# ankitkumar93/compute-war

Measured on AMD Instinct MI355X. Metric: GB/s ingested (Skein-512 + LZ4, 64 KiB blocks), higher is better.
Workload: dtype u64; 1 GPU; skein512+lz4, 1048576 x 65536 B uniform-random blocks/GPU in HBM; blocks_per_gpu=1048576, block_bytes=65536, parallelism=block-sharded x1, gather-only RCCL

## Files before the change

compute_war_amd/csrc/lz4_kernel.hip:

```cpp

#include <hip/hip_runtime.h>
#include <stdint.h>
#include <stdio.h>
#include <stdlib.h>
#include <string.h>

#include <mutex>
#include <type_traits>
#include <unordered_map>

#include "cw_device.h"
#include "lz_device.h"

#ifndef HEADW_GLOBAL
#define HEADW_GLOBAL 16
#endif
#ifndef HEADW_STAGED
#define HEADW_STAGED 64
#endif

namespace cw {

using lz::Around;
using lz::around;
// ... 188 lines not shown
struct Chunk { uint4 p[kPieces]; };

__device__ __forceinline__ void chunk_load(Chunk &r, const uint8_t *g, uint32_t c, uint32_t nchunks, uint32_t n, uint32_t lane)
{
#pragma unroll
    for (uint32_t j = 0; j < kPieces; j++) {
        const uint32_t off = c * kChunk + j * 1024 + lane * 16;
        if (c < nchunks && off < n) r.p[j] = *reinterpret_cast<const uint4 *>(g + off);
    }
}
__device__ __forceinline__ void chunk_stage(const Chunk &r, uint32_t *ring32, uint32_t c, uint32_t n, uint32_t lane)
{
#pragma unroll
    for (uint32_t j = 0; j < kPieces; j++) {
        const uint32_t off = c * kChunk + j * 1024 + lane * 16;
        if (off < n) *reinterpret_cast<uint4 *>(reinterpret_cast<uint8_t *>(ring32) + (off & (kRing - 1))) = r.p[j];
    }
}
__device__ __forceinline__ void chunk_store(const Chunk &r, uint8_t *lit, uint32_t c, uint32_t n, uint32_t lane)
{
#pragma unroll
    for (uint32_t j = 0; j < kPieces; j++) {
        const uint32_t off = c * kChunk + j * 1024 + lane * 16;
        if (off < n) {
            uint32_t *q = reinterpret_cast<uint32_t *>(lit + off);
            __builtin_nontemporal_store(r.p[j].x, q);
            __builtin_nontemporal_store(r.p[j].y, q + 1);
            __builtin_nontemporal_store(r.p[j].z, q + 2);
            __builtin_nontemporal_store(r.p[j].w, q + 3);
        }
    }
}

struct Walk {
    ScanState st;
    uint32_t knext = 0, v0 = 0;
    bool marked = false;
};

template <int NG>
__device__ __forceinline__ void probe_groups(Walk &w, const uint32_t (&pos)[kStreamGroup], const bool (&act)[kStreamGroup], uint32_t *tab,
                                             const uint32_t *ring32, uint32_t tag, uint32_t epoch)
{
    uint32_t v[NG], old[NG];
#pragma unroll
    for (int j = 0; j < NG; j++) {
        const uint32_t a0 = (pos[j] & (kRing - 1)) >> 2, a1 = (a0 + 1) & (kRing / 4 - 1);
        v[j] = __builtin_amdgcn_alignbyte(ring32[a1], ring32[a0], pos[j] & 3u);
    }
#pragma unroll
    for (int j = 0; j < NG; j++) old[j] = scan_issue(tab, tag, pos[j], v[j], act[j]);
#pragma unroll
    for (int j = 0; j < NG; j++) scan_judge(old[j], epoch, w.v0, pos[j], v[j], act[j], w.st);
}

__device__ __forceinline__ void probe_upto(Walk &w, uint32_t end, uint32_t *tab, const uint32_t *ring32, uint32_t tag, uint32_t epoch,
                                           uint32_t nprobes, const uint8_t *g, uint32_t lane)
{
    for (;;) {
        uint32_t pos[kStreamGroup], nact = 0, ngroups = 0;
        bool act[kStreamGroup];
#pragma unroll
        for (uint32_t j = 0; j < kStreamGroup; j++) {
            const uint32_t k = w.knext + 64 * j + lane;
            pos[j] = 1 + probe_delta(k);
            act[j] = k < nprobes && pos[j] < end;
            const unsigned long long m = __ballot(act[j]);
            nact += (uint32_t)__builtin_popcountll(m);
            ngroups += m != 0;
        }
        if (nact == 0) return;
        if (ngroups == 1) probe_groups<1>(w, pos, act, tab, ring32, tag, epoch);
        else if (ngroups == 2) probe_groups<2>(w, pos, act, tab, ring32, tag, epoch);
        else probe_groups<kStreamGroup>(w, pos, act, tab, ring32, tag, epoch);
        w.marked = scan_settle(g, w.st);
        w.knext += nact;
        if (w.marked || nact < 64 * kStreamGroup) return;
    }
}

__global__ void __launch_bounds__(64)
lz4_scan_stream_kernel(const uint8_t *__restrict__ src, uint32_t n, size_t src_stride, size_t nblocks,
                       uint8_t *__restrict__ dst, size_t dst_stride, uint32_t *__restrict__ sizes, uint32_t nprobes,
                       uint32_t *__restrict__ queue, uint32_t *__restrict__ counters, size_t first_block, uint32_t feed_word)
{
    __shared__ __attribute__((aligned(16))) uint32_t tab[1u << 13];
    __shared__ __attribute__((aligned(16))) uint32_t ring32[kRing / 4];
    volatile uint32_t *mailbox = ring32;
    const uint32_t lane = threadIdx.x;
    __builtin_amdgcn_s_setprio(3);
    uint32_t epoch = 15;
    const uint32_t nchunks = (n + kChunk - 1) / kChunk;
    const uint32_t hdr = 1 + (n >= 15 ? (n - 15) / 255 + 1 : 0);

    BlockFeed feed;
    const uint32_t run = n >= 65536 ? 1u : 65536u / n;
    for (size_t rel; scan_next_block(feed, rel, counters + feed_word - 2, mailbox, run, nblocks - first_block, lane);) {
        const size_t blk = first_block + rel;
        scan_begin_block(tab, epoch, lane);
        const uint8_t *g = src + blk * src_stride;
        uint8_t *out = dst + blk * dst_stride, *lit = out + hdr;
        const uint32_t tag = epoch << 28;
        Walk w;
        Chunk r0, r1, r2;

#define CW_STAGE(PREV, CUR, C)                                                                         \
        do {                                                                                           \
            const uint32_t c_ = (C);                                                                   \
            if (c_) chunk_store(PREV, lit, c_ - 1, n, lane);                                           \
            chunk_load(PREV, g, c_ + 2, nchunks, n, lane);                                             \
            chunk_stage(CUR, ring32, c_, n, lane);                                                     \
            if (c_ == 0) {                                                                             \
                w.v0 = ring32[0];                                                                      \
                if (nprobes && lane == 0) {                                                            \
                    const uint32_t h0 = w.v0 * 2654435761u;                                            \
                    atomicMax(&tab[h0 >> 19], tag | ((h0 >> 7) & 0xFFFu));             \
                }                                                                                      \
            } else {                                                                                   \
                probe_upto(w, c_ * kChunk, tab, ring32, tag, epoch, nprobes, g, lane);                 \
            }                                                                                          \
        } while (0)

        chunk_load(r0, g, 0, nchunks, n, lane);
        chunk_load(r1, g, 1, nchunks, n, lane);
        for (uint32_t c = 0; c < nchunks && !w.marked; c += 3) {
            CW_STAGE(r2, r0, c);
            if (c + 1 < nchunks && !w.marked) CW_STAGE(r0, r1, c + 1);
            if (c + 2 < nchunks && !w.marked) CW_STAGE(r1, r2, c + 2);
        }
#undef CW_STAGE
        if (!w.marked) {
            probe_upto(w, n, tab, ring32, tag, epoch, nprobes, g, lane);
            if (!w.marked) {
                const uint32_t last = (nchunks - 1) % 3;
                if (last == 0) chunk_store(r0, lit, nchunks - 1, n, lane);
                else if (last == 1) chunk_store(r1, lit, nchunks - 1, n, lane);
                else chunk_store(r2, lit, nchunks - 1, n, lane);
            }
        }
        if (w.marked) {
            scan_mark(sizes, blk, queue, counters, lane);
            continue;
        }
        if (n >= 15) {
            if (lane == 0) out[0] = 15u << 4;
            put_len(out + 1, n - 15, lane);
        } else if (lane == 0) {
            out[0] = (uint8_t)(n << 4);
        }
        if (lane == 0) sizes[blk] = hdr + n;
    }
}

#ifdef CW_CLOCK_STAMP
__device__ unsigned long long g_clock_scan[4 * kClockSlots];
hipError_t lz4_clock_read(unsigned long long *out) { return hipMemcpyFromSymbol(out, HIP_SYMBOL(g_clock_scan), sizeof g_clock_scan); }
#endif

__global__ void __launch_bounds__(64)
lz4_scan_span_kernel(const uint8_t *__restrict__ src, uint32_t n, size_t src_stride, uint32_t nspans, uint8_t *__restrict__ dst,
                     size_t dst_stride, uint32_t *__restrict__ sizes, uint32_t nprobes, uint32_t *__restrict__ queue,
                     uint32_t *__restrict__ counters, uint32_t lg)
{
    CW_CLOCK_SCOPE(g_clock_scan);
    __shared__ __attribute__((aligned(16))) uint32_t tab[1u << 13];
    __shared__ __attribute__((aligned(16))) uint32_t ring32[kRing / 4];
    volatile uint32_t *mailbox = ring32;
    const uint32_t lane = threadIdx.x;
    __builtin_amdgcn_s_setprio(3);
    uint32_t epoch = 15;
    const uint32_t cmask = (1u << lg) - 1, run = 16u >> lg;
    const uint32_t hdr = 1 + (n - 15) / 255 + 1;
    const uint32_t lane16 = lane * 16;

    for (;;) {
        __syncthreads();
        if (lane == 0) *mailbox = atomicAdd(&counters[2], 1u);
        __syncthreads();
        const uint32_t span = __builtin_amdgcn_readfirstlane(*mailbox);
        if (span >= nspans) break;
        __syncthreads();
        const size_t first = (size_t)span * run;
        const uint8_t *gs = src + first * src_stride;
        uint8_t *os = dst + first * dst_stride + hdr;

        Walk w;
        size_t blk = first;
        uint32_t tag = 0, marks = 0;
        Chunk r0, r1, r2;
#define CW_LD(R, I)                                                                                          \
        do {                                                                                                 \
            const uint32_t i_ = (I) < 15u ? (I) : 15u;                                                       \
            const uint8_t *p_ = gs + (size_t)(i_ >> lg) * src_stride + ((i_ & cmask) << 12) + lane16;        \
            _Pragma("unroll") for (uint32_t j = 0; j < kPieces; j++) R.p[j] = *reinterpret_cast<const uint4 *>(p_ + j * 1024); \
        } while (0)
#define CW_ST(R, I)                                                                                          \
        do {                                                                                                 \
            const uint32_t i_ = (I);                                                                         \
            uint8_t *p_ = os + (size_t)(i_ >> lg) * dst_stride + ((i_ & cmask) << 12) + lane16;              \
            _Pragma("unroll") for (uint32_t j = 0; j < kPieces; j++) {                                       \
                uint32_t *q = reinterpret_cast<uint32_t *>(p_ + j * 1024);  \
                __builtin_nontemporal_store(R.p[j].x, q);     __builtin_nontemporal_store(R.p[j].y, q + 1);  \
                __builtin_nontemporal_store(R.p[j].z, q + 2); __builtin_nontemporal_store(R.p[j].w, q + 3);  \
            }                                                                                                \
        } while (0)
#define CW_FINISH()                                                                                          \
        do {                      \
            if (!w.marked) probe_upto(w, n, tab, ring32, tag, epoch, nprobes, src + blk * src_stride, lane); \
            if (w.marked) marks |= 1u << (uint32_t)(blk - first);         \
            else {                                                                                           \
                uint8_t *out = dst + blk * dst_stride;                                                       \
                if (lane == 0) out[0] = 15u << 4;                                                            \
                put_len(out + 1, n - 15, lane);                                                              \
                if (lane == 0) sizes[blk] = hdr + n;                                                         \
            }                                                                                                \
        } while (0)
#define CW_BEGIN(I)                                                                                          \
        do {                                                                                                 \
            blk = first + ((I) >> lg);                                                                       \
            scan_begin_block(tab, epoch, lane);                                                              \
            tag = epoch << 28;                                                                               \
            w = Walk();                                                                                      \
        } while (0)
#define CW_STAGE_IN(R, C)                                                                                    \
        do {                                                                                                 \
            uint8_t *p_ = reinterpret_cast<uint8_t *>(ring32) + (((C) & 1u) << 12) + lane16;                 \
            _Pragma("unroll") for (uint32_t j = 0; j < kPieces; j++) *reinterpret_cast<uint4 *>(p_ + j * 1024) = R.p[j]; \
        } while (0)
#define CW_AFTER_STAGE(C)                                                                                    \
        do {                                                                                                 \
            if ((C) == 0) {                                                                                  \
                w.v0 = ring32[0];                                                                            \
                if (nprobes && lane == 0) {                                                                  \
                    const uint32_t h0 = w.v0 * 2654435761u;                                                  \
                    atomicMax(&tab[h0 >> 19], tag | ((h0 >> 7) & 0xFFFu));                   \
                }                                                                                            \
            } else if (!w.marked) {                                                                          \
                probe_upto(w, (C) * kChunk, tab, ring32, tag, epoch, nprobes, src + blk * src_stride, lane); \
            }                                                                                                \
        } while (0)
#define CW_STEP(PREV, CUR, I)                                                                                \
        do {                                                                                                 \
            const uint32_t s_ = (I), c_ = s_ & cmask;                                                        \
            CW_ST(PREV, s_ - 1);                                                                             \
            CW_LD(PREV, s_ + 2);                                                                             \
            if (c_ == 0) { CW_FINISH(); CW_BEGIN(s_); }                                                      \
            CW_STAGE_IN(CUR, c_);                                                                            \
            CW_AFTER_STAGE(c_);                                                                              \
        } while (0)

        CW_LD(r0, 0u);
        CW_LD(r1, 1u);
        CW_LD(r2, 2u);
        CW_BEGIN(0u);
        CW_STAGE_IN(r0, 0u);
        CW_AFTER_STAGE(0u);
        for (uint32_t i = 1; i < 16; i += 3) {
            CW_STEP(r0, r1, i);
            CW_STEP(r1, r2, i + 1);
            CW_STEP(r2, r0, i + 2);
        }
        CW_ST(r0, 15u);
        CW_FINISH();
        if (marks) {
            uint32_t base = 0;
            if (lane == 0) base = atomicAdd(&counters[1], (uint32_t)__builtin_popcount(marks));
            base = __builtin_amdgcn_readfirstlane(base);
            if (lane < 16 && ((marks >> lane) & 1u)) {
                sizes[first + lane] = kNeedsParse;
                queue[base + (uint32_t)__builtin_popcount(marks & ((1u << lane) - 1u))] = (uint32_t)(first + lane);
            }
        }
#undef CW_LD
#undef CW_ST
#undef CW_FINISH
#undef CW_BEGIN
#undef CW_STAGE_IN
#undef CW_AFTER_STAGE
#undef CW_STEP
    }
}

static uint32_t scan_probes(uint32_t n)
{
    if (n < kMFLimit + 1) return 0;
    const uint32_t limit = n - 11;
    uint32_t k = 0, p = 1, step = 1, nb = 64;
    while (p + step <= limit) { p += step; step = nb++ >> 6; k++; }
    return k;
}

template <bool STAGED>
__global__ void __launch_bounds__(64)
lz4_blocks_kernel(const uint8_t *__restrict__ src, uint32_t n, size_t src_stride, size_t nblocks,
                  uint8_t *__restrict__ dst, size_t dst_stride, uint32_t *__restrict__ sizes,
                  const uint32_t *__restrict__ queue, uint32_t *__restrict__ counters)
{
    extern __shared__ __attribute__((aligned(16))) uint8_t smem[];
    uint16_t *tab = reinterpret_cast<uint16_t *>(smem);
    uint8_t *lds_in = smem + kTabBytes;
    const uint32_t lane = threadIdx.x;

    const uint32_t qcount = counters[1];
    volatile uint32_t *mailbox = reinterpret_cast<volatile uint32_t *>(tab);
    for (uint32_t guard = 0; guard <= qcount; guard++) {
        __syncthreads();
        if (lane == 0) *mailbox = atomicAdd(&counters[0], 1u);
        __syncthreads();
        const uint32_t qi = __builtin_amdgcn_readfirstlane(*mailbox);
        if (qi >= qcount) break;
        const size_t blk = queue[qi];
        const uint8_t *g = src + blk * src_stride;
        uint8_t *out = dst + blk * dst_stride;

        __syncthreads();
        const uint8_t *in = STAGED ? lds_in : g;
        if (STAGED) {
            if ((reinterpret_cast<uintptr_t>(g) & 15) == 0) {
                const uint4 *g4 = reinterpret_cast<const uint4 *>(g);
                const uint32_t nvec = n >> 4;
                for (uint32_t i = lane; i < nvec; i += 64) reinterpret_cast<uint4 *>(lds_in)[i] = g4[i];
                for (uint32_t i = (nvec << 4) + lane; i < n; i += 64) lds_in[i] = g[i];
            } else {
                for (uint32_t i = lane; i < n; i += 64) lds_in[i] = g[i];
            }
        }
        for (uint32_t i = lane; i < kTabBytes / 16; i += 64) reinterpret_cast<uint4 *>(tab)[i] = make_uint4(0, 0, 0, 0);
        __syncthreads();

        uint32_t ip = 0, anchor = 0, op = 0;

        if (n >= kMFLimit + 1) {
            const uint32_t mflimit = n - kMFLimit, matchlimit = n - kLastLiterals;
            uint32_t ins = 0, s0 = 1;
            bool has_retest = false;

            for (uint32_t seq = 0; seq < n; seq++) {
                uint32_t match = 0, mpos = 0;
                bool found = false, exhausted = false;
                for (uint32_t t0 = 0;;) {
                    const uint32_t t = t0 + lane, k = t - 2;
                    const bool is_probe = t >= 2;
                    const uint32_t dk = t0 == 0 ? k : probe_delta(k), stepk = k == 0 ? 1u : (63u + k) >> 6;
                    const uint32_t pos = t == 0 ? ins : t == 1 ? ip : s0 + dk;
                    const bool dead = is_probe && s0 + dk + stepk > mflimit + 1;
                    const bool active = !dead && (is_probe || t == 0 || has_retest);
                    const uint32_t ndead = ctz64(__ballot(dead));
                    const unsigned long long amask = __ballot(active);
                    if (!amask) { exhausted = true; break; }

                    uint32_t v = 0, h = 0, old = 0;
                    if (active) {
                        v = rd32x<STAGED>(in, pos);
                        h = hash13(v);
                        old = tab[h];
                        tab[h] = (uint16_t)pos;
                    }
                    __syncthreads();
                    const bool lost = active && (tab[h] != (uint16_t)pos);
                    const uint32_t fa = ctz64(amask);
                    uint32_t m = ctz64(__ballot(lost));
                    if (m == fa) m = fa + 1;
                    const uint32_t L = m < ndead ? m : ndead;

                    const bool eq = active && t != 0 && lane < L && rd32x<STAGED>(in, old) == v;
                    const unsigned long long eqmask = __ballot(eq);
                    const uint32_t ncommit = eqmask ? ctz64(eqmask) + 1 : L;
                    if (__ballot(active && lane >= ncommit)) {
                        if (active && lane >= ncommit) tab[h] = (uint16_t)old;
                        if (active && lane < ncommit) tab[h] = (uint16_t)pos;
                    }
                    if (eqmask) {
                        const uint32_t w = ctz64(eqmask);
                        mpos = __builtin_amdgcn_readlane(pos, w);
                        match = __builtin_amdgcn_readlane(old, w);
                        found = true;
                        break;
                    }
                    if (ndead < 64 && L == ndead) { exhausted = true; break; }
                    t0 += L;
                }
                (void)exhausted;
                if (!found) break;
                ip = mpos;

                uint32_t mc, back;
                {
                    bool ok;
                    if (lane < 48) {
                        const uint32_t i = ip + kMinMatch + lane;
                        ok = i < matchlimit && in[i] == in[match + kMinMatch + lane];
// ... 1083 lines not shown
            state = LB_NEXT;
        }
    }
}

template <int K>
__global__ void __launch_bounds__(64)
lz4_lanes_ring_kernel(const uint8_t *__restrict__ src, uint32_t n, size_t src_stride, uint8_t *__restrict__ dst, size_t dst_stride,
                      uint32_t *__restrict__ sizes, const uint32_t *__restrict__ queue, uint32_t *__restrict__ counters,
                      uint16_t *__restrict__ tables, uint32_t min_blocks, uint32_t reserve, uint32_t max_blocks)
{
    __shared__ uint32_t ring[(kRingBytes / 4) * 64];
    const uint32_t qcount = counters[1];
    if (qcount < min_blocks || qcount >= max_blocks) return;
    if ((size_t)blockIdx.x * 64 >= qcount) return;
    lz4_lanes_ring_body<K>(ring, qcount, src, n, src_stride, dst, dst_stride, sizes, queue, counters, tables, reserve);
}

__global__ void __launch_bounds__(64)
lz4_lanes_ring_auto_kernel(const uint8_t *__restrict__ src, uint32_t n, size_t src_stride, uint8_t *__restrict__ dst, size_t dst_stride,
                           uint32_t *__restrict__ sizes, const uint32_t *__restrict__ queue, uint32_t *__restrict__ counters,
                           uint16_t *__restrict__ tables, uint32_t min_blocks, uint32_t reserve_mid, uint32_t wide_from, uint32_t reserve_wide,
                           uint32_t leave_mid)
{
    __shared__ uint32_t ring[(kRingBytes / 4) * 64];
    const uint32_t qcount = counters[1];
    if (qcount < min_blocks) return;
    if ((size_t)blockIdx.x * 64 >= qcount) return;
    if (qcount >= wide_from) {
        lz4_lanes_ring_body<1>(ring, qcount, src, n, src_stride, dst, dst_stride, sizes, queue, counters, tables, reserve_wide);
    } else {
        if ((size_t)blockIdx.x * 64 + leave_mid >= qcount && blockIdx.x > 0) return;
        lz4_lanes_ring_body<2>(ring, qcount, src, n, src_stride, dst, dst_stride, sizes, queue, counters, tables, reserve_mid);
    }
}

namespace {
struct Workspace {
    uint32_t *p = nullptr; size_t cap = 0;
    uint16_t *lane_tabs = nullptr; size_t lane_cap = 0;
    hipStream_t side = nullptr; hipEvent_t fork = nullptr, join = nullptr;
    hipStream_t side2 = nullptr; hipEvent_t fork2 = nullptr, join2 = nullptr;
    std::mutex launch;
};
std::mutex ws_lock;
std::unordered_map<uint64_t, Workspace> ws_map;

Workspace &find_workspace(hipStream_t stream)
{
    std::lock_guard<std::mutex> g(ws_lock);
    return ws_map[ws_key(stream)];
}

hipError_t grow_workspace(Workspace &w, size_t nblocks, uint32_t **out, size_t *cap_out)
{
    if (w.cap < nblocks) {
        if (w.p) { hipError_t e = hipFree(w.p); if (e != hipSuccess) return e; }
        w.p = nullptr; w.cap = 0;
        size_t cap = nblocks < 4096 ? 4096 : nblocks;
        hipError_t e = hipMalloc(reinterpret_cast<void **>(&w.p), (2 * cap + 8) * sizeof(uint32_t));
        if (e != hipSuccess) return e;
        w.cap = cap;
    }
    *out = w.p;
    *cap_out = w.cap;
    return hipSuccess;
}
}

const uint32_t *lz4_queued_blocks_word(hipStream_t stream)
{
    std::lock_guard<std::mutex> g(ws_lock);
    auto it = ws_map.find(ws_key(stream));
    return it == ws_map.end() || !it->second.p ? nullptr : it->second.p + 1;
}

void lz4_release_workspaces()
{
    std::lock_guard<std::mutex> g(ws_lock);
    for (auto &kv : ws_map) {
        if (kv.second.p) (void)hipFree(kv.second.p);
        if (kv.second.lane_tabs) (void)hipFree(kv.second.lane_tabs);
        if (kv.second.side) { (void)hipStreamDestroy(kv.second.side); (void)hipEventDestroy(kv.second.fork); (void)hipEventDestroy(kv.second.join); }
        if (kv.second.side2) { (void)hipStreamDestroy(kv.second.side2); (void)hipEventDestroy(kv.second.fork2); (void)hipEventDestroy(kv.second.join2); }
    }
    ws_map.clear();
}

void lz4_release_stream(hipStream_t stream)
{
    std::lock_guard<std::mutex> g(ws_lock);
    auto it = ws_map.find(ws_key(stream));
    if (it == ws_map.end()) return;
    Workspace &w = it->second;
    if (w.p) (void)hipFree(w.p);
    if (w.lane_tabs) (void)hipFree(w.lane_tabs);
    if (w.side) { (void)hipStreamDestroy(w.side); (void)hipEventDestroy(w.fork); (void)hipEventDestroy(w.join); }
    if (w.side2) { (void)hipStreamDestroy(w.side2); (void)hipEventDestroy(w.fork2); (void)hipEventDestroy(w.join2); }
    ws_map.erase(it);
}

hipError_t lz4_launch(const uint8_t *src, size_t block_bytes, size_t src_stride, size_t nblocks, uint8_t *dst,
                      size_t dst_stride, uint32_t *sizes, hipStream_t stream, const AfterScan *after_scan)
{
    if (nblocks == 0) return hipSuccess;
    if (block_bytes == 0 || block_bytes > 65536 || nblocks > 0xFFFFFFFFull) return hipErrorInvalidValue;
    const uint32_t n = (uint32_t)block_bytes;
    const char *sm_env = tune("CW_LZ4_STAGE_MAX");
    const uint32_t stage_max = sm_env && atoi(sm_env) >= 0 ? (uint32_t)atoi(sm_env) : 4096u;
    const bool staged = n <= (stage_max < kStageMax ? stage_max : kStageMax);
    uint32_t lds = kTabBytes + (staged ? ((n + 15u) & ~15u) + (n % 4 ? 16u : 0u) : 0u);
    static bool attr_set = false;
    if (!attr_set) {
        hipError_t e = hipFuncSetAttribute(reinterpret_cast<const void *>(lz4_blocks_kernel<true>),
                                           hipFuncAttributeMaxDynamicSharedMemorySize, kStageMax + kTabBytes + 16);
        if (e != hipSuccess) return e;
        e = hipFuncSetAttribute(reinterpret_cast<const void *>(lz4_parse_kernel<true>),
                                hipFuncAttributeMaxDynamicSharedMemorySize, kStageMax + kTabBytes + 16);
        if (e != hipSuccess) return e;
        attr_set = true;
    }
    uint32_t *ws = nullptr;
    size_t cap = 0;
    Workspace &wsp = find_workspace(stream);
    std::lock_guard<std::mutex> sequence(wsp.launch);
    hipError_t e = grow_workspace(wsp, nblocks, &ws, &cap);
    if (e != hipSuccess) return e;
    uint32_t *counters = ws, *queue = ws + 8, *queue2 = ws + 8 + cap;
    char launched[320] = "";
    auto note = [&](const char *fmt, auto... a) __attribute__((format(printf, 2, 0))) {
        const size_t used = strlen(launched);
        if (used && used + 3 < sizeof launched) strcat(launched, " + ");
        const size_t at = strlen(launched);
#pragma clang diagnostic push
#pragma clang diagnostic ignored "-Wformat-security"
        snprintf(launched + at, sizeof launched - at, fmt, a...);
#pragma clang diagnostic pop
    };

    if ((e = hipMemsetAsync(counters, 0, 8 * sizeof(uint32_t), stream)) != hipSuccess) return e;
    const char *mode = tune("CW_LZ4_MODE");
    const size_t scan_grid = nblocks < 256 * 5 ? nblocks : 256 * 5;
    const bool streamable = ((reinterpret_cast<uintptr_t>(src) | src_stride | n) & 15) == 0 && !(mode && strcmp(mode, "generic") == 0);
    if (streamable) {
        const char *wpc_env = tune("CW_SCAN_WPC");
        const size_t wpc = wpc_env && atoi(wpc_env) > 0 ? (size_t)atoi(wpc_env) : 4;
        const bool pow2 = n >= kChunk && (n & (n - 1)) == 0 && !(mode && strcmp(mode, "stream") == 0);
        uint32_t lg = 0;
        while (pow2 && (kChunk << lg) < n) lg++;
        const size_t run = pow2 ? (size_t)(16u >> lg) : 1;
        const size_t nspans = pow2 ? nblocks / run : 0, done = nspans * run;
        if (nspans) {
            const size_t g = nspans < 256 * wpc ? nspans : 256 * wpc;
            hipLaunchKernelGGL(lz4_scan_span_kernel, dim3((unsigned)g), dim3(64), 0, stream, src, n, src_stride, (uint32_t)nspans, dst,
                               dst_stride, sizes, scan_probes(n), queue, counters, lg);
            note("cw::lz4_scan_span_kernel");
        }
        if (done < nblocks) {
            const size_t rest = nblocks - done;
            const size_t sgrid = rest < 256 * wpc ? rest : 256 * wpc;
            hipLaunchKernelGGL(lz4_scan_stream_kernel, dim3((unsigned)sgrid), dim3(64), 0, stream, src, n, src_stride, nblocks, dst,
                               dst_stride, sizes, scan_probes(n), queue, counters, done, 3u);
            note("cw::lz4_scan_stream_kernel");
        }
    } else {
        hipLaunchKernelGGL(lz4_scan_kernel, dim3((unsigned)scan_grid), dim3(64), 0, stream, src, n, src_stride, nblocks, dst,
                           dst_stride, sizes, scan_probes(n), queue, counters);
        note("cw::lz4_scan_kernel");
    }
    if ((e = hipGetLastError()) != hipSuccess) return e;
    if (after_scan && (e = after_scan->fn(after_scan->ctx)) != hipSuccess) return e;
    if (mode && strcmp(mode, "scan") == 0) { note_kernels(0, launched); return hipSuccess; }
    const char *gen_env = tune("CW_LZ4_PARSE");
    const bool use_fp = !staged && gen_env && strcmp(gen_env, "fp") == 0;
    const char *hw_env = tune("CW_LZ4_HEADW");
    const int headw = hw_env ? atoi(hw_env) : 16;
    if (use_fp) lds = kTabBytes + kFpBytes;
    const size_t per_cu = (160u * 1024u) / lds ? (160u * 1024u) / lds : 1;
    const char *lanes_env = tune("CW_LZ4_LANES");
    const uint32_t lane_min = lanes_env ? (uint32_t)atoi(lanes_env)
                              : staged ? kLaneMinSmall : n > 32768 ? kLaneMidBlocks : n > 16384 ? 40960u : n > 8192 ? 61440u : 98304u;
    bool lanes_used = false, lanes_beside = false;
    const char *lf_env = tune("CW_LZ4_LANES_FP");
    const bool lanes_fp = !(lf_env && lf_env[0] == '0');
    const char *lr_env = tune("CW_LZ4_LANES_RING");
    const int lanes_ring = lr_env ? atoi(lr_env) : -1;
    if (!use_fp && lane_min && nblocks >= lane_min && n >= 64) {
        const char *lw_env = tune("CW_LANES_WPC");
        const size_t lwpc = lw_env && atoi(lw_env) > 0 ? (size_t)atoi(lw_env) : 8;
        size_t lgrid = (nblocks + 63) / 64, lcap = 256 * lwpc;
        uint32_t lane_leave = 0;
        if (staged && !(lw_env && atoi(lw_env) > 0)) lcap = nblocks / 128 < 512 ? 512 : nblocks / 128 > 2048 ? 2048 : nblocks / 128;
        if (lgrid > lcap) lgrid = lcap;
        const char *ll_env = tune("CW_LANES_LEAVE");
        const size_t leave = ll_env ? (size_t)atoi(ll_env) : kLaneLeave;
        if (!staged && leave && !(tune("CW_LANES_CONCURRENT") && tune("CW_LANES_CONCURRENT")[0] == '0') && lane_min > 1) {
            lane_leave = (uint32_t)leave;
            const size_t want = nblocks > leave + 4096 ? (nblocks - leave + 63) / 64 : 64;
            if (nblocks < kLaneWideBlocks && lgrid > want) lgrid = want;
        }
        if (wsp.lane_cap < lgrid * 64) {
            if (wsp.lane_tabs) { e = hipFree(wsp.lane_tabs); if (e != hipSuccess) return e; }
            wsp.lane_tabs = nullptr; wsp.lane_cap = 0;
            e = hipMalloc(reinterpret_cast<void **>(&wsp.lane_tabs), lgrid * 64 * (size_t)kTabBytes * 2);
            if (e != hipSuccess) {
                (void)hipGetLastError();
                wsp.lane_tabs = nullptr;
                lgrid = 0;
            } else {
                wsp.lane_cap = lgrid * 64;
            }
        }
        if (lgrid) {
        const char *cc_env = tune("CW_LANES_CONCURRENT");
        const char *rs_env = tune("CW_LANES_RESERVE");
        lanes_beside = cc_env ? cc_env[0] != '0' : true;
        uint32_t reserve = 0, reserve_wide = 0, lmin = lane_min;
        if (lanes_beside) {
            if (!wsp.side) {
                {
                    const char *sp_env = tune("CW_SIDE_PRIO");
                    int least = 0, greatest = 0;
                    if ((e = hipDeviceGetStreamPriorityRange(&least, &greatest)) != hipSuccess) return e;
                    e = !(sp_env && sp_env[0] == '0') ? hipStreamCreateWithPriority(&wsp.side, hipStreamNonBlocking, greatest)
                                                   : hipStreamCreateWithFlags(&wsp.side, hipStreamNonBlocking);
                    if (e != hipSuccess) return e;
                }
                if ((e = hipEventCreateWithFlags(&wsp.fork, hipEventDisableTiming)) != hipSuccess) return e;
                if ((e = hipEventCreateWithFlags(&wsp.join, hipEventDisableTiming)) != hipSuccess) return e;
            }
            reserve = rs_env && atoi(rs_env) > 0 ? (uint32_t)atoi(rs_env) : (staged ? 32768u : kLaneShare);
            if (!staged && !(rs_env && atoi(rs_env) > 0) && reserve > nblocks / 3 * 2) reserve = (uint32_t)(nblocks / 3 * 2);
            reserve_wide = rs_env && atoi(rs_env) > 0 ? (uint32_t)atoi(rs_env) : kLaneShareWide;
            if (lane_min > 1 && lmin < reserve + reserve / 4) lmin = reserve + reserve / 4;
            if (lane_min == 1) reserve = reserve_wide = 0;
            if ((e = hipEventRecord(wsp.fork, stream)) != hipSuccess) return e;
            if ((e = hipStreamWaitEvent(wsp.side, wsp.fork, 0)) != hipSuccess) return e;
        }
        hipStream_t ls = lanes_beside ? wsp.side : stream;
        const uint32_t no_max = 0xFFFFFFFFu;
        const char *side_tag = lanes_beside ? " [side stream]" : "";
#define CW_RING(K, LO, HI) do { \
            const uint32_t lo_ = (LO), hi_ = (HI); \
            hipLaunchKernelGGL(lz4_lanes_ring_kernel<K>, dim3((unsigned)lgrid), dim3(64), 0, ls, src, n, src_stride, dst, dst_stride, sizes, queue, counters, \
                               wsp.lane_tabs, lo_, hi_ == no_max && lanes_ring < 0 ? reserve_wide : reserve, hi_); \
            if (hi_ == no_max) note("cw::lz4_lanes_ring_kernel<" #K "> (queue >= %u)%s", lo_, side_tag); \
            else note("cw::lz4_lanes_ring_kernel<" #K "> (queue in [%u, %u))%s", lo_, hi_, side_tag); } while (0)
        if (n <= 4096)
        {
            hipLaunchKernelGGL(lz4_lanes_kernel<kLaneTagged>, dim3((unsigned)lgrid), dim3(64), 0, ls, src, n, src_stride, dst, dst_stride, sizes, queue,
                               counters, wsp.lane_tabs, lmin, reserve);
            note("cw::lz4_lanes_kernel<1> (queue >= %u)%s", lmin, side_tag);
        }
        else if (lanes_ring < 0) {
            const uint32_t wide_from = lmin < kLaneWideBlocks ? kLaneWideBlocks : lmin;
            hipLaunchKernelGGL(lz4_lanes_ring_auto_kernel, dim3((unsigned)lgrid), dim3(64), 0, ls, src, n, src_stride, dst, dst_stride, sizes, queue, counters,
                               wsp.lane_tabs, lmin, reserve, wide_from, reserve_wide, lane_leave);
            note("cw::lz4_lanes_ring_auto_kernel (queue >= %u: two positions per iteration, >= %u: one)%s", lmin, wide_from, side_tag);
        }
        else if (lanes_ring == 1) CW_RING(1, lmin, no_max);
        else if (lanes_ring == 2) CW_RING(2, lmin, no_max);
        else if (lanes_ring == 4) CW_RING(4, lmin, no_max);
        else if (lanes_ring == 8) CW_RING(8, lmin, no_max);
#undef CW_RING
        else if (lanes_fp) {
            hipLaunchKernelGGL(lz4_lanes_kernel<kLaneFp>, dim3((unsigned)lgrid), dim3(64), 0, ls, src, n, src_stride, dst, dst_stride, sizes, queue,
                               counters, wsp.lane_tabs, lmin, reserve);
            note("cw::lz4_lanes_kernel<2> (queue >= %u)%s", lmin, side_tag);
        } else {
            hipLaunchKernelGGL(lz4_lanes_kernel<kLanePlain>, dim3((unsigned)lgrid), dim3(64), 0, ls, src, n, src_stride, dst, dst_stride, sizes, queue,
                               counters, wsp.lane_tabs, lmin, reserve);
            note("cw::lz4_lanes_kernel<0> (queue >= %u)%s", lmin, side_tag);
        }
        if ((e = hipGetLastError()) != hipSuccess) return e;
        lanes_used = true;
        }
    }
    const char *vt_env = tune("CW_LZ4_VTAB");
    const int vt_mode = vt_env ? atoi(vt_env) : 2;
    const bool cut_first = mode && strcmp(mode, "cut") == 0;
    bool vtab_used = false, vtab_beside = false;
    if (vt_mode > 0 && !use_fp && !cut_first && n >= 64 && nblocks >= 64 && ((reinterpret_cast<uintptr_t>(src) | src_stride) & 3) == 0) {
        const char *vm_env = tune("CW_VTAB_MIN"), *vx_env = tune("CW_VTAB_MAX"), *vr_env = tune("CW_VTAB_RESERVE"), *vw_env = tune("CW_VTAB_WPC");
        const uint32_t vmin = vm_env ? (uint32_t)atoi(vm_env) : staged ? 12288u : 1u, vres = vr_env ? (uint32_t)atoi(vr_env) : 0u;
        const uint32_t vmax = vx_env ? (uint32_t)atoi(vx_env) : (lanes_used && !lanes_beside ? lane_min : 0xFFFFFFFFu);
        const unsigned vwpc = vw_env && atoi(vw_env) > 0 ? (unsigned)atoi(vw_env) : 16u;
        hipStream_t vs = stream;
        if (vt_mode == 2) {
            if (!wsp.side2) {
                {
                    const char *sp_env = tune("CW_SIDE_PRIO");
                    int least = 0, greatest = 0;
                    if ((e = hipDeviceGetStreamPriorityRange(&least, &greatest)) != hipSuccess) return e;
                    e = !(sp_env && sp_env[0] != '2') ? hipStreamCreateWithPriority(&wsp.side2, hipStreamNonBlocking, greatest)
                                                   : hipStreamCreateWithFlags(&wsp.side2, hipStreamNonBlocking);
                    if (e != hipSuccess) return e;
                }
                if ((e = hipEventCreateWithFlags(&wsp.fork2, hipEventDisableTiming)) != hipSuccess) return e;
                if ((e = hipEventCreateWithFlags(&wsp.join2, hipEventDisableTiming)) != hipSuccess) return e;
            }
            if ((e = hipEventRecord(wsp.fork2, stream)) != hipSuccess) return e;
            if ((e = hipStreamWaitEvent(wsp.side2, wsp.fork2, 0)) != hipSuccess) return e;
            vs = wsp.side2;
            vtab_beside = true;
        }
        const char *vname = nullptr;
        if ((e = lz4_vtab_launch(src, n, src_stride, nblocks, dst, dst_stride, sizes, queue, counters, vmin, vmax, vres, vwpc, vs, &vname)) != hipSuccess) return e;
        if (vmax != 0xFFFFFFFFu) note("%s (queue < %u)%s", vname, vmax, vtab_beside ? " [side stream]" : "");
        else note("%s%s", vname, vtab_beside ? " [side stream]" : "");
// ... 59 lines not shown
```

Baseline: 1103 GB/s.

## Align literal stores to 16 bytes and batch hash probes in LZ4 span scan

Adds an ALIGNED variant of the span scan kernel. When dst is 16-byte aligned, the output is shifted back by two bytes so each lane's literal copy becomes full 16-byte nontemporal vector stores, built with alignbyte from the previous word in the LDS ring. The header is written as aligned vector stores as well. Hash-table probing is replaced by a batched probe_range that handles 64 or 128 probe positions per wave with ballots, and per-chunk probe end indices are precomputed via binary search. The aim is to cut unaligned byte and dword store traffic and probe loop overhead, at the cost of extra LDS reads and more complex edge handling for the first and last two bytes.

```diff
diff --git a/compute_war_amd/csrc/lz4_kernel.hip b/compute_war_amd/csrc/lz4_kernel.hip
--- a/compute_war_amd/csrc/lz4_kernel.hip
+++ b/compute_war_amd/csrc/lz4_kernel.hip
@@ -364,11 +364,94 @@
     }
 }
 
+__device__ __forceinline__ uint32_t probe_pos(uint32_t k)
+{
+    const uint32_t q = (k + 62) >> 6;
+    return q * (k + 31 - 32 * q) + 1 + (uint32_t)(k != 0);
+}
+
+__device__ __forceinline__ uint32_t probe_kend(uint32_t end, uint32_t nprobes)
+{
+    uint32_t lo = 0, hi = nprobes;
+    while (lo < hi) {
+        const uint32_t mid = (lo + hi) >> 1;
+        if (probe_pos(mid) < end) lo = mid + 1;
+        else hi = mid;
+    }
+    return lo;
+}
+
+template <int NG, bool PART>
+__device__ __forceinline__ bool probe_batches(uint32_t kb, uint32_t rem, uint32_t *tab, const uint32_t *ring32, uint32_t tag, uint32_t v0,
+                                              const uint8_t *g, uint32_t lane)
+{
+    uint32_t pos[NG], v[NG], tp[NG], fp[NG], old[NG];
+    unsigned long long actm[NG];
+#pragma unroll
+    for (int j = 0; j < NG; j++) {
+        pos[j] = probe_pos(kb + 64 * j + lane);
+        const uint8_t *r8 = reinterpret_cast<const uint8_t *>(ring32);
+        const uint32_t lo = *reinterpret_cast<const uint32_t *>(r8 + (pos[j] & (kRing - 4)));
+        const uint32_t hi = *reinterpret_cast<const uint32_t *>(r8 + ((pos[j] + 4) & (kRing - 4)));
+        v[j] = __builtin_amdgcn_alignbyte(hi, lo, pos[j]);
+    }
+#pragma unroll
+    for (int j = 0; j < NG; j++) {
+        const bool act = !PART || 64 * j + lane < rem;
+        actm[j] = PART ? __ballot(act) : ~0ull;
+        const uint32_t h = v[j] * 2654435761u;
+        fp[j] = (h >> 7) & 0xFFFu;
+        tp[j] = tag | (pos[j] << 12);
+        old[j] = atomicMax(&tab[act ? h >> 19 : 0u], act ? tp[j] | fp[j] : 0u);
+    }
+    unsigned long long hit = 0, maybe = 0;
+#pragma unroll
+    for (int j = 0; j < NG; j++) {
+        const unsigned long long empty = __ballot(old[j] < tag);
+        hit |= (__ballot(old[j] >= tp[j]) | (empty & __ballot(v[j] == v0))) & actm[j];
+        const unsigned long long fm = __ballot(((old[j] ^ fp[j]) & 0xFFFu) == 0) & ~empty & actm[j];
+        hit |= fm & maybe;
+        maybe |= fm;
+    }
+    if (maybe) {
+        uint32_t mcand = 0, mv = 0;
+#pragma unroll
+        for (int j = 0; j < NG; j++) {
+            const bool f = (((PART ? actm[j] : ~0ull) >> lane) & 1u) && old[j] >= tag && ((old[j] ^ fp[j]) & 0xFFFu) == 0;
+            mcand = f ? (old[j] >> 12) & 0xFFFFu : mcand;
+            mv = f ? v[j] : mv;
+        }
+        const bool mine = (maybe >> lane) & 1u;
+        hit |= __ballot(mine && ld32g(g + mcand) == mv);
+    }
+    return hit != 0;
+}
+
+__device__ __forceinline__ void store16_nt(uint8_t *p, uint32_t x, uint32_t y, uint32_t z, uint32_t w)
+{
+    typedef uint32_t u32x4 __attribute__((ext_vector_type(4)));
+    u32x4 v = {x, y, z, w};
+    __builtin_nontemporal_store(v, reinterpret_cast<u32x4 *>(p));
+}
+
+__device__ __forceinline__ void probe_range(Walk &w, uint32_t ke, uint32_t *tab, const uint32_t *ring32, uint32_t tag, const uint8_t *g,
+                                            uint32_t lane)
+{
+    uint32_t kb = w.knext;
+    for (; kb + 128 <= ke; kb += 128)
+        if (probe_batches<2, false>(kb, 0, tab, ring32, tag, w.v0, g, lane)) { w.marked = true; return; }
+    const uint32_t rem = ke - kb;
+    if (rem > 64) w.marked = probe_batches<2, true>(kb, rem, tab, ring32, tag, w.v0, g, lane);
+    else if (rem) w.marked = probe_batches<1, true>(kb, rem, tab, ring32, tag, w.v0, g, lane);
+    w.knext = ke;
+}
+
 #ifdef CW_CLOCK_STAMP
 __device__ unsigned long long g_clock_scan[4 * kClockSlots];
 hipError_t lz4_clock_read(unsigned long long *out) { return hipMemcpyFromSymbol(out, HIP_SYMBOL(g_clock_scan), sizeof g_clock_scan); }
 #endif
 
+template <bool ALIGNED>
 __global__ void __launch_bounds__(64)
 lz4_scan_span_kernel(const uint8_t *__restrict__ src, uint32_t n, size_t src_stride, uint32_t nspans, uint8_t *__restrict__ dst,
                      size_t dst_stride, uint32_t *__restrict__ sizes, uint32_t nprobes, uint32_t *__restrict__ queue,
@@ -384,6 +467,8 @@
     const uint32_t cmask = (1u << lg) - 1, run = 16u >> lg;
     const uint32_t hdr = 1 + (n - 15) / 255 + 1;
     const uint32_t lane16 = lane * 16;
+    const uint32_t kend = probe_kend(lane * kChunk, nprobes);
+    const uint32_t hdrw = (0xFFu << 16) | (((n - 15) % 255) << 24);
 
     for (;;) {
         __syncthreads();
@@ -394,7 +479,7 @@
         __syncthreads();
         const size_t first = (size_t)span * run;
         const uint8_t *gs = src + first * src_stride;
-        uint8_t *os = dst + first * dst_stride + hdr;
+        uint8_t *os = dst + first * dst_stride + (ALIGNED ? hdr - 2 : hdr);
 
         Walk w;
         size_t blk = first;
@@ -408,22 +493,42 @@
         } while (0)
 #define CW_ST(R, I)                                                                                          \
         do {                                                                                                 \
-            const uint32_t i_ = (I);                                                                         \
-            uint8_t *p_ = os + (size_t)(i_ >> lg) * dst_stride + ((i_ & cmask) << 12) + lane16;              \
-            _Pragma("unroll") for (uint32_t j = 0; j < kPieces; j++) {                                       \
-                uint32_t *q = reinterpret_cast<uint32_t *>(p_ + j * 1024);  \
-                __builtin_nontemporal_store(R.p[j].x, q);     __builtin_nontemporal_store(R.p[j].y, q + 1);  \
-                __builtin_nontemporal_store(R.p[j].z, q + 2); __builtin_nontemporal_store(R.p[j].w, q + 3);  \
+            const uint32_t i_ = (I), c_ = i_ & cmask;                                                        \
+            uint8_t *p_ = os + (size_t)(i_ >> lg) * dst_stride + (c_ << 12) + lane16;                        \
+            if constexpr (ALIGNED) {                                                                         \
+                const uint32_t b_ = ((c_ & 1u) << 12) + lane16;  \
+                uint32_t pw_[kPieces];                                                                       \
+                _Pragma("unroll") for (uint32_t j = 0; j < kPieces; j++) pw_[j] = ring32[((b_ + j * 1024 - 4) & (kRing - 4)) / 4]; \
+                if (c_ == 0 && lane == 0) pw_[0] = hdrw;                                                     \
+                _Pragma("unroll") for (uint32_t j = 0; j < kPieces; j++) {                                   \
+                    store16_nt(p_ + j * 1024, __builtin_amdgcn_alignbyte(R.p[j].x, pw_[j], 2),               \
+                               __builtin_amdgcn_alignbyte(R.p[j].y, R.p[j].x, 2),                            \
+                               __builtin_amdgcn_alignbyte(R.p[j].z, R.p[j].y, 2),                            \
+                               __builtin_amdgcn_alignbyte(R.p[j].w, R.p[j].z, 2));                           \
+                }                                                                                            \
+                if (c_ == cmask && lane == 63)                                 \
+                    *reinterpret_cast<uint16_t *>(p_ + (kPieces - 1) * 1024 + 16) = (uint16_t)(R.p[kPieces - 1].w >> 16); \
+            } else {                                                                                         \
+                _Pragma("unroll") for (uint32_t j = 0; j < kPieces; j++) {                                   \
+                    uint32_t *q = reinterpret_cast<uint32_t *>(p_ + j * 1024);  \
+                    __builtin_nontemporal_store(R.p[j].x, q);     __builtin_nontemporal_store(R.p[j].y, q + 1); \
+                    __builtin_nontemporal_store(R.p[j].z, q + 2); __builtin_nontemporal_store(R.p[j].w, q + 3); \
+                }                                                                                            \
             }                                                                                                \
         } while (0)
 #define CW_FINISH()                                                                                          \
         do {                      \
-            if (!w.marked) probe_upto(w, n, tab, ring32, tag, epoch, nprobes, src + blk * src_stride, lane); \
+            if (!w.marked) probe_range(w, nprobes, tab, ring32, tag, src + blk * src_stride, lane);          \
             if (w.marked) marks |= 1u << (uint32_t)(blk - first);         \
             else {                                                                                           \
                 uint8_t *out = dst + blk * dst_stride;                                                       \
-                if (lane == 0) out[0] = 15u << 4;                                                            \
-                put_len(out + 1, n - 15, lane);                                                              \
+                if constexpr (ALIGNED) {                                                                     \
+                    if (lane < (hdr - 2) / 16)                                                               \
+                        store16_nt(out + lane16, lane ? ~0u : 0xFFFFFFF0u, ~0u, ~0u, ~0u);                   \
+                } else {                                                                                     \
+                    if (lane == 0) out[0] = 15u << 4;                                                        \
+                    put_len(out + 1, n - 15, lane);                                                          \
+                }                                                                                            \
                 if (lane == 0) sizes[blk] = hdr + n;                                                         \
             }                                                                                                \
         } while (0)
@@ -448,7 +553,7 @@
                     atomicMax(&tab[h0 >> 19], tag | ((h0 >> 7) & 0xFFFu));                   \
                 }                                                                                            \
             } else if (!w.marked) {                                                                          \
-                probe_upto(w, (C) * kChunk, tab, ring32, tag, epoch, nprobes, src + blk * src_stride, lane); \
+                probe_range(w, __builtin_amdgcn_readlane(kend, (C)), tab, ring32, tag, src + blk * src_stride, lane); \
             }                                                                                                \
         } while (0)
 #define CW_STEP(PREV, CUR, I)                                                                                \
@@ -1838,9 +1943,16 @@
         const size_t nspans = pow2 ? nblocks / run : 0, done = nspans * run;
         if (nspans) {
             const size_t g = nspans < 256 * wpc ? nspans : 256 * wpc;
-            hipLaunchKernelGGL(lz4_scan_span_kernel, dim3((unsigned)g), dim3(64), 0, stream, src, n, src_stride, (uint32_t)nspans, dst,
-                               dst_stride, sizes, scan_probes(n), queue, counters, lg);
-            note("cw::lz4_scan_span_kernel");
+            const bool aligned = ((reinterpret_cast<uintptr_t>(dst) | dst_stride) & 15) == 0;
+            if (aligned) {
+                hipLaunchKernelGGL(lz4_scan_span_kernel<true>, dim3((unsigned)g), dim3(64), 0, stream, src, n, src_stride, (uint32_t)nspans,
+                                   dst, dst_stride, sizes, scan_probes(n), queue, counters, lg);
+                note("cw::lz4_scan_span_kernel<true>");
+            } else {
+                hipLaunchKernelGGL(lz4_scan_span_kernel<false>, dim3((unsigned)g), dim3(64), 0, stream, src, n, src_stride, (uint32_t)nspans,
+                                   dst, dst_stride, sizes, scan_probes(n), queue, counters, lg);
+                note("cw::lz4_scan_span_kernel<false>");
+            }
         }
         if (done < nblocks) {
             const size_t rest = nblocks - done;
```

Result: faster. 1145 GB/s, median of 6 (+3.9%).
